# Enigmatisms/NeRF

Measured on AMD Instinct MI355X. Metric: rays/s (64+128 samples), 800x800, higher is better.
Workload: dtype bf16

## Files before the change

### nerf_amd/csrc/sample_kernels.hip

```cpp
#include "device_common.h"
#include "host_common.h"
#include "../../include/nerf_amd.h"

extern __shared__ __attribute__((aligned(16))) char smem[];

namespace {

constexpr int WAVES_PER_BLOCK = 4;

DEVINL int wave_in_block() { return (int)(threadIdx.x >> 6); }

constexpr int ENC_TILE = 64;
static inline size_t enc_lds_bytes(int L) { return (size_t)ENC_TILE * (6 * L + 6) * 4; }
template <bool IPE, class Moments>
DEVINL void encode_tile(float (*mom)[6], float* stage, int64_t base, int64_t total, int L, float* __restrict__ feat, Moments&& moments) {
    const int width = 6 * L, pairs_per = 3 * L;
    const int nsamp = (int)(total - base < ENC_TILE ? total - base : ENC_TILE);
    if ((int)threadIdx.x < nsamp) moments((int)threadIdx.x, base + threadIdx.x);
    __syncthreads();
    const int n_pairs = nsamp * pairs_per;
    for (int p = threadIdx.x; p < n_pairs; p += blockDim.x) {
        const int sl = p / pairs_per, rem = p - sl * pairs_per;
        const int l = rem / 3, c = rem - 3 * l;
        float sn, cs;
// ... 219 lines not shown
    for (int64_t n0 = blockIdx.x * (int64_t)4; n0 < N; n0 += (int64_t)gridDim.x * 4) {
        __syncthreads();
        if (threadIdx.x < 4 && n0 + threadIdx.x < N) {
            const int64_t n = n0 + threadIdx.x;
            const int64_t cell = (int64_t)__umul64hi(sampler_index_word(n, seed), P);
            const int64_t k = cell / wp, r = cell - k * wp;
            const int64_t wr = r / ww;
            const int64_t row = y0 + wr, col = x0 + (r - wr * ww);
            const int64_t v = view_ids != nullptr ? view_ids[k] : k;
            float* q = ray_s[threadIdx.x];
            if (v >= 0 && v < V) {
                sampler_ray(poses + v * 12, fx, fy, (float)(col - W / 2), (float)(H / 2 - row), q, rays + n * 6);
                const float* px = images + ((v * 3) * (int64_t)H + row) * W + col;
#pragma unroll
                for (int c = 0; c < 3; ++c) rgb[n * 3 + c] = px[(int64_t)c * H * W];
                if (index != nullptr) index[n] = (v * H + row) * W + col;
            } else {
                const float nan = __builtin_nanf("");
#pragma unroll
                for (int c = 0; c < 6; ++c) { q[c] = nan; rays[n * 6 + c] = nan; }
#pragma unroll
                for (int c = 0; c < 3; ++c) rgb[n * 3 + c] = nan;
                if (index != nullptr) index[n] = -1;
            }
        }
        __syncthreads();
        if (lengths == nullptr) continue;
        sampler_samples(n0, N, C, seed, near, res, ray_s, lengths, pts);
    }
}

__global__ void length2pts_kernel(const float* __restrict__ rays, const float* __restrict__ z, int64_t N, int S,
                                  float* __restrict__ out) {
    const int64_t total = N * S * 6;
    for (int64_t i = blockIdx.x * (int64_t)blockDim.x + threadIdx.x; i < total; i += (int64_t)gridDim.x * blockDim.x) {
        const int64_t ns = i / 6;
        const int k = (int)(i - ns * 6);
        const int64_t n = ns / S;
        const float* r = rays + n * 6;
        out[i] = (k < 3) ? (r[k] + r[3 + k] * z[ns]) : r[k];
    }
}

__global__ __launch_bounds__(256) void sigma_to_weights_kernel(const float* __restrict__ sigma, const float* __restrict__ z,
                                                              const float* __restrict__ dirs, int64_t N, int S, int act,
                                                              float* __restrict__ w) {
    for (int64_t n = blockIdx.x * (int64_t)WAVES_PER_BLOCK + wave_in_block(); n < N; n += (int64_t)gridDim.x * WAVES_PER_BLOCK) {
        float nrm = 1.0f;
        const bool scale = dirs != nullptr;
        if (scale) nrm = norm3(dirs[n * 3], dirs[n * 3 + 1], dirs[n * 3 + 2]);
        const float* sg = sigma + n * S;
        const float* zz = z + n * S;
        float* wo = w + n * S;
        wave_sigma_to_weights(S, act, [&](int s) { return sg[s]; },
                              [&](int s) { return scale ? zz[s] * nrm : zz[s]; },
                              [&](int s, float wv, float) { wo[s] = wv; });
    }
}

__global__ void max_blur_kernel(const float* __restrict__ w, int64_t N, int S, float alpha, float* __restrict__ out) {
    const int64_t total = N * S;
    for (int64_t i = blockIdx.x * (int64_t)blockDim.x + threadIdx.x; i < total; i += (int64_t)gridDim.x * blockDim.x) {
        const int s = (int)(i % S);
        const float c = w[i];
        const float front = (s == 0) ? c : fmaxf(w[i - 1], c);
        const float rear = (s == S - 1) ? c : fmaxf(c, w[i + 1]);
        out[i] = 0.5f * (front + rear) + alpha;
    }
}

DEVINL void lds_wave_sync() {
    __builtin_amdgcn_fence(__ATOMIC_RELEASE, "workgroup");
    __builtin_amdgcn_wave_barrier();
    __builtin_amdgcn_fence(__ATOMIC_ACQUIRE, "workgroup");
}

#ifndef SORT_NB_DEF
#define SORT_NB_DEF 256
#define SORT_CAP_DEF 6
#endif
constexpr int SORT_NB = SORT_NB_DEF, SORT_CAP = SORT_CAP_DEF, SORT_PER_LANE = SORT_NB / 64;
constexpr int SORT_LDS_FLOATS = 2 * SORT_NB + SORT_NB * SORT_CAP / 2;

template <class UF>
DEVINL void wave_inverse_sample(const float* pw, const float* bins, int nw, float* cdf, float* samp, int* bel, int* sortbuf,
                                UF&& uf, int K, int sort, float* __restrict__ z_out,
                                int64_t* __restrict__ below_out, int64_t* __restrict__ above_out) {
    const int lane = lane_id();
    const int nb = nw + 1;
    float* part8 = reinterpret_cast<float*>(sortbuf);
    const int nv = nw >> 3;
    if (lane < 8) {
        const int n4 = nv >> 2;
        float a0 = 0.0f, a1 = 0.0f, a2 = 0.0f, a3 = 0.0f;
        for (int i = 0; i < n4; ++i) {
            a0 += pw[32 * i + lane] + 1e-5f;
            a1 += pw[32 * i + 8 + lane] + 1e-5f;
            a2 += pw[32 * i + 16 + lane] + 1e-5f;
            a3 += pw[32 * i + 24 + lane] + 1e-5f;
        }
        for (int v = 4 * n4; v < nv; ++v) a0 += pw[8 * v + lane] + 1e-5f;
        a0 += a1; a0 += a2; a0 += a3;
        part8[lane] = a0;
    }
    lds_wave_sync();
    float total = 0.0f;
    if (nv > 0) {
        for (int j = 8 * nv; j < nw; ++j) total += pw[j] + 1e-5f;
#pragma unroll
        for (int c = 0; c < 8; ++c) total += part8[c];
    } else {
        float a1 = 0.0f, a2 = 0.0f, a3 = 0.0f;
        if (nw >= 4) { total += pw[0] + 1e-5f; a1 += pw[1] + 1e-5f; a2 += pw[2] + 1e-5f; a3 += pw[3] + 1e-5f; }
        for (int j = nw & ~3; j < nw; ++j) total += pw[j] + 1e-5f;
        total += a1; total += a2; total += a3;
    }
    double carry = 0.0;
    if (lane == 0) cdf[0] = 0.0f;
    for (int base = 0; base < nw; base += 64) {
        const int j = base + lane;
        double p = 0.0;
        if (j < nw) p = (double)((pw[j] + 1e-5f) / total);
        const double incl = wave_incl_scan_add(p);
        if (j < nw) cdf[1 + j] = (float)(carry + incl);
        carry += wave_last(incl);
    }
    lds_wave_sync();
    const int halvings = 32 - __builtin_clz((unsigned)nb);
    for (int k0 = 0, i0 = 0; k0 < K; k0 += 192, i0 += 3) {
        float uu[3]; int lo[3], hi[3];
#pragma unroll
        for (int q = 0; q < 3; ++q) {
            const int k = k0 + 64 * q + lane;
            uu[q] = (k < K) ? uf(i0 + q, k) : 0.0f;
            lo[q] = 0; hi[q] = (k < K) ? nb : 0;
        }
        for (int it = 0; it < halvings; ++it) {
#pragma unroll
            for (int q = 0; q < 3; ++q) {
                const int mid = (lo[q] + hi[q]) >> 1;
                const bool open_ = lo[q] < hi[q];
                const float c = cdf[open_ ? mid : 0];
                if (open_) { if (c <= uu[q]) lo[q] = mid + 1; else hi[q] = mid; }
            }
        }
#pragma unroll
        for (int q = 0; q < 3; ++q) {
            const int k = k0 + 64 * q + lane;
            if (k >= K) continue;
            const int below = lo[q] - 1 > 0 ? lo[q] - 1 : 0;
            const int above = lo[q] < nb - 1 ? lo[q] : nb - 1;
            const float c0 = cdf[below], c1 = cdf[above];
            float denom = c1 - c0;
            if (denom < 1e-5f) denom = 1.0f;
            const float t = (uu[q] - c0) / denom;
            const float b0 = bins[below], b1 = bins[above];
            const float v = b0 + t * (b1 - b0);
            if (sort) { samp[k] = v; bel[k] = below; }
            else {
                z_out[k] = v;
                if (below_out) below_out[k] = below;
                if (above_out) above_out[k] = above;
            }
        }
    }
    if (!sort) return;
    lds_wave_sync();
    int* cnt = sortbuf;
    int* pre = sortbuf + SORT_NB;
    unsigned short* mem = reinterpret_cast<unsigned short*>(sortbuf + 2 * SORT_NB);
    for (int b = lane; b < SORT_NB; b += 64) cnt[b] = 0;
    lds_wave_sync();
    int overflow = 0;
    for (int j = lane; j + 1 < nb; j += 64) overflow |= (bins[j + 1] < bins[j]) ? 1 : 0;
    for (int k = lane, i = 0; k < K; k += 64, ++i) {
        int b = (int)(uf(i, k) * (float)SORT_NB);
        b = b < 0 ? 0 : (b > SORT_NB - 1 ? SORT_NB - 1 : b);
        const int pos = atomicAdd(&cnt[b], 1);
        if (pos < SORT_CAP) mem[b * SORT_CAP + pos] = (unsigned short)k; else overflow = 1;
    }
    lds_wave_sync();
    if (__any(overflow)) {
        for (int k = lane; k < K; k += 64) {
            const float v = samp[k];
            int rank = 0;
            for (int j = 0; j < K; ++j) {
                const float o = samp[j];
                rank += (o < v || (o == v && j < k)) ? 1 : 0;
            }
            z_out[rank] = v;
            if (below_out) below_out[rank] = bel[k];
        }
        return;
    }
    {
        int c[SORT_PER_LANE], tot = 0;
#pragma unroll
        for (int i = 0; i < SORT_PER_LANE; ++i) { c[i] = cnt[lane * SORT_PER_LANE + i]; tot += c[i]; }
        int run = wave_incl_scan_add(tot) - tot;
#pragma unroll
        for (int i = 0; i < SORT_PER_LANE; ++i) { pre[lane * SORT_PER_LANE + i] = run; run += c[i]; }
    }
    lds_wave_sync();
    for (int k0 = 0, i0 = 0; k0 < K; k0 += 192, i0 += 3) {
        float v[3]; int rank[3], cntb[3], bb[3];
#pragma unroll
        for (int q = 0; q < 3; ++q) {
            const int k = k0 + 64 * q + lane;
            const bool ok = k < K;
            int b = ok ? (int)(uf(i0 + q, k) * (float)SORT_NB) : 0;
            b = b < 0 ? 0 : (b > SORT_NB - 1 ? SORT_NB - 1 : b);
            bb[q] = b;
            v[q] = samp[ok ? k : 0];
            rank[q] = pre[b];
            cntb[q] = ok ? cnt[b] : 0;
        }
        int most = cntb[0] > cntb[1] ? cntb[0] : cntb[1];
        most = most > cntb[2] ? most : cntb[2];
        const int trips = wave_max_i(most);
        for (int p = 0; p < trips; ++p) {
#pragma unroll
            for (int q = 0; q < 3; ++q) {
                const int k = k0 + 64 * q + lane;
                const bool live = p < cntb[q];
                const int jx = mem[bb[q] * SORT_CAP + p];
                const float o = samp[live ? jx : 0];
                rank[q] += (live && (o < v[q] || (o == v[q] && jx < k))) ? 1 : 0;
            }
        }
#pragma unroll
        for (int q = 0; q < 3; ++q) {
            const int k = k0 + 64 * q + lane;
            if (k >= K) continue;
            z_out[rank[q]] = v[q];
            if (below_out) below_out[rank[q]] = bel[k];
        }
    }
}

DEVINL size_t inv_lds_floats(int C, int K) { return (size_t)3 * C + 2 * K + SORT_LDS_FLOATS; }

__global__ __launch_bounds__(256) void inverse_sample_kernel(const float* __restrict__ w, const float* __restrict__ z,
                                                            const float* __restrict__ u, int64_t N, int C, int K, int sort,
                                                            int mode, float* __restrict__ z_out, int64_t* __restrict__ below,
                                                            int64_t* __restrict__ above) {
    float* base = reinterpret_cast<float*>(smem) + wave_in_block() * inv_lds_floats(C, K);
    float* pw = base; float* bins = pw + C; float* cdf = bins + C; float* samp = cdf + C;
    int* bel = reinterpret_cast<int*>(samp + K);
    int* sortbuf = bel + K;
    const int lane = lane_id();
    const int nw = mode == 0 ? C - 2 : C - 1;
    const int wstride = mode == 0 ? C : C - 1;
    for (int64_t n = blockIdx.x * (int64_t)WAVES_PER_BLOCK + wave_in_block(); n < N; n += (int64_t)gridDim.x * WAVES_PER_BLOCK) {
        lds_wave_sync();
        if (mode == 0) {
            for (int j = lane; j < nw; j += 64) pw[j] = w[n * wstride + 1 + j];
            for (int j = lane; j < nw + 1; j += 64) bins[j] = 0.5f * (z[n * C + j + 1] + z[n * C + j]);
        } else {
            for (int j = lane; j < nw; j += 64) pw[j] = w[n * wstride + j];
            for (int j = lane; j < nw + 1; j += 64) bins[j] = z[n * C + j];
        }
        lds_wave_sync();
        const float* un = u + n * K;
        wave_inverse_sample(pw, bins, nw, cdf, samp, bel, sortbuf, [&](int, int k) { return un[k]; }, K, sort, z_out + n * K,
                            below ? below + n * K : nullptr, above ? above + n * K : nullptr);
    }
}

struct ResampleArgs {
    const float* density; const float* z; const float* z_base; const float* u_strat; float z_jitter;
    const float* dirs; int dirs_stride; const float* u_inv; int64_t N; int C; int K; int softplus; float alpha;
    float* z_fine; int64_t* below; float* w_prop; float* z_coarse;
    uint64_t rng_seed; int64_t rng_ray_offset;
};

#ifndef RS_BLOCKS_PER_CU
#define RS_BLOCKS_PER_CU 5
#endif
__global__ __launch_bounds__(256) __attribute__((amdgpu_waves_per_eu(RS_BLOCKS_PER_CU, RS_BLOCKS_PER_CU))) void resample_kernel(ResampleArgs a) {
    const int C = a.C, K = a.K;
    float* base = reinterpret_cast<float*>(smem) + wave_in_block() * (inv_lds_floats(C, K) + 2 * C);
    float* pw = base; float* bins = pw + C; float* cdf = bins + C; float* samp = cdf + C;
    int* bel = reinterpret_cast<int*>(samp + K);
    int* sortbuf = bel + K;
    float* zl = reinterpret_cast<float*>(sortbuf + SORT_LDS_FLOATS);
    float* wraw = zl + C;
    const int lane = lane_id();
    struct RayIn { float dx, dy, dz, zv0, zv1, dens0, dens1, u0, u1, u2; };
    const bool fits = C <= 128 && K <= 192;
    auto load_in = [&](int64_t n) -> RayIn {
        RayIn r;
        const float* dd = a.dirs + n * a.dirs_stride;
        r.dx = dd[0]; r.dy = dd[1]; r.dz = dd[2];
        Philox4 blk = {{0u, 0u, 0u, 0u}};
        const bool draw = !a.u_inv || (!a.z && !a.u_strat);
        if (draw) blk = philox_ray_block(a.rng_seed, n + a.rng_ray_offset, lane);
        auto depth_of = [&](int j, bool first) {
            if (a.z) return a.z[n * C + j];
            const float uu = a.u_strat ? a.u_strat[n * C + j] : (first ? u01_from_bits(blk.w[0]) : philox_u_strat(a.rng_seed, n + a.rng_ray_offset, j));
            return a.z_base[j] + uu * a.z_jitter;
        };
        r.zv0 = r.zv1 = r.dens0 = r.dens1 = 0.0f;
        if (lane < C) { r.zv0 = depth_of(lane, true); r.dens0 = a.density[n * C + lane]; }
        if (lane + 64 < C) { r.zv1 = depth_of(lane + 64, false); r.dens1 = a.density[n * C + lane + 64]; }
        if (a.u_inv) {
            const float* un = a.u_inv + n * K;
            r.u0 = (lane < K) ? un[lane] : 0.0f;
            r.u1 = (lane + 64 < K) ? un[lane + 64] : 0.0f;
            r.u2 = (lane + 128 < K) ? un[lane + 128] : 0.0f;
        } else {
            r.u0 = u01_from_bits(blk.w[1]); r.u1 = u01_from_bits(blk.w[2]); r.u2 = u01_from_bits(blk.w[3]);
        }
        return r;
    };
    const int64_t stride = (int64_t)gridDim.x * WAVES_PER_BLOCK;
    int64_t n = blockIdx.x * (int64_t)WAVES_PER_BLOCK + wave_in_block();
    if (n >= a.N) return;
    RayIn cur = {};
    if (fits) cur = load_in(n);
    for (; n < a.N; n += stride) {
        RayIn nxt = cur;
        if (fits && n + stride < a.N) nxt = load_in(n + stride);
        lds_wave_sync();
        float nrm;
        if (fits) {
            nrm = norm3(cur.dx, cur.dy, cur.dz);
            if (lane < C) { zl[lane] = cur.zv0; if (a.z_coarse) a.z_coarse[n * C + lane] = cur.zv0; }
            if (lane + 64 < C) { zl[lane + 64] = cur.zv1; if (a.z_coarse) a.z_coarse[n * C + lane + 64] = cur.zv1; }
        } else {
            const float* dd = a.dirs + n * a.dirs_stride;
            nrm = norm3(dd[0], dd[1], dd[2]);
            for (int j = lane; j < C; j += 64) {
                const float zv = a.z ? a.z[n * C + j]
                                     : (a.z_base[j] + (a.u_strat ? a.u_strat[n * C + j] : philox_u_strat(a.rng_seed, n + a.rng_ray_offset, j)) * a.z_jitter);
                zl[j] = zv;
                if (a.z_coarse) a.z_coarse[n * C + j] = zv;
            }
        }
        lds_wave_sync();
        const float* sg = a.density + n * C;
        const int soft = a.softplus;
        const float dens0 = cur.dens0, dens1 = cur.dens1, cu0 = cur.u0, cu1 = cur.u1, cu2 = cur.u2;
        wave_sigma_to_weights(C, NERF_AMD_ACT_RELU,
                              [=](int s) { const float d = fits ? ((s >> 6) ? dens1 : dens0) : sg[s]; return soft ? softplus_f(d) : d; },
                              [=](int s) { return zl[s] * nrm; },
                              [=](int s, float wv, float) { wraw[s] = wv; });
        lds_wave_sync();
        for (int j = lane; j < C; j += 64) {
            const float c = wraw[j];
            const float front = (j == 0) ? c : fmaxf(wraw[j - 1], c);
            const float rear = (j == C - 1) ? c : fmaxf(c, wraw[j + 1]);
            const float wb = 0.5f * (front + rear) + a.alpha;
            if (j >= 1 && j <= C - 2) pw[j - 1] = wb;
            if (a.w_prop) a.w_prop[n * C + j] = wb;
        }
        for (int j = lane; j < C - 1; j += 64) bins[j] = 0.5f * (zl[j + 1] + zl[j]);
        lds_wave_sync();
        const float* un = a.u_inv ? a.u_inv + n * K : nullptr;
        const uint64_t seed = a.rng_seed; const int64_t nn = n + a.rng_ray_offset;
        wave_inverse_sample(pw, bins, C - 2, cdf, samp, bel, sortbuf,
                            [=](int i, int k) {
                                if (fits) return i == 0 ? cu0 : (i == 1 ? cu1 : cu2);
                                if (un) return un[k];
                                return philox_u_inv(seed, nn, k);
                            },
                            K, 1, a.z_fine + n * K, a.below ? a.below + n * K : nullptr, nullptr);
        cur = nxt;
    }
}

struct CompositeArgs {
    const float* rgbo; const float* z; int z_stride; const float* dirs; int dirs_stride; int64_t N; int S;
    int flags; int act; float sigma_shift; float near, far; const float* normal; const float* cam_dir;
    float* rgb; float* weights; float* depth; float* normal_img;
};

template <int NCH>
struct RayRecs { f32x4 c[NCH]; float z[NCH]; float dx, dy, dz; };
template <int NCH>
DEVINL RayRecs<NCH> load_ray(const CompositeArgs& a, int64_t n, int lane) {
    RayRecs<NCH> r;
    const f32x4 zero = {0.0f, 0.0f, 0.0f, 0.0f};
    const f32x4* px = reinterpret_cast<const f32x4*>(a.rgbo) + n * a.S;
    const float* zz = a.z + n * a.z_stride;
    const float* dd = a.dirs + n * a.dirs_stride;
#pragma unroll
    for (int k = 0; k < NCH; ++k) {
        const int s = 64 * k + lane;
        r.c[k] = (s < a.S) ? px[s] : zero;
        r.z[k] = (s < a.S) ? zz[s] : 0.0f;
    }
    r.dx = dd[0]; r.dy = dd[1]; r.dz = dd[2];
    return r;
}
template <int NCH>
DEVINL void composite_ray_fast(const CompositeArgs& a, int64_t n, const RayRecs<NCH>& r, int lane) {
    const int S = a.S;
    const bool mul = (a.flags & 1) != 0;
    const float nrm = mul ? norm3(r.dx, r.dy, r.dz) : 1.0f;
    float zn[NCH];
#pragma unroll
    for (int k = 0; k < NCH; ++k) zn[k] = mul ? r.z[k] * nrm : r.z[k];
    float accr = 0.0f, accg = 0.0f, accb = 0.0f, accw = 0.0f, accd = 0.0f;
    double carry = 1.0;
    float* wout = a.weights ? a.weights + n * S : nullptr;
#pragma unroll
    for (int k = 0; k < NCH; ++k) {
        if (k > 0 && 64 * k >= S) break;
        const int s = 64 * k + lane;
        float nx = __shfl_down(zn[k], 1, 64);
        if (k + 1 < NCH) { const float first = __shfl(zn[k + 1 < NCH ? k + 1 : k], 0, 64); if (lane == 63) nx = first; }
        float w = 0.0f;
        double p = 1.0;
        if (s < S) {
            const float delta = (s + 1 < S) ? (nx - zn[k]) : 1e10f;
            const float m = expf(-density_act(r.c[k][3] + a.sigma_shift, a.act) * delta);
            w = 1.0f - m; p = (double)(m + 1e-10f);
        }
        const double incl = wave_incl_scan_mul(p);
        const double excl = wave_shift_up1(incl, 1.0);
        w *= (float)(carry * excl);
        carry *= wave_last(incl);
        if (s < S) {
            accr += w * r.c[k][0]; accg += w * r.c[k][1]; accb += w * r.c[k][2]; accw += w; accd += w * zn[k];
            if (wout) wout[s] = w;
        }
    }
    accr = wave_sum(accr); accg = wave_sum(accg); accb = wave_sum(accb); accw = wave_sum(accw); accd = wave_sum(accd);
    if (lane == 0) {
        if (a.flags & 2) { const float bg = 1.0f - accw; accr += bg; accg += bg; accb += bg; }
        a.rgb[n * 3] = accr; a.rgb[n * 3 + 1] = accg; a.rgb[n * 3 + 2] = accb;
        if (a.depth) a.depth[n] = (accd - a.near) / (a.far - a.near);
    }
}
template <int NCH>
DEVINL void composite_rays_fast(const CompositeArgs& a, int lane) {
    const int64_t stride = (int64_t)gridDim.x * WAVES_PER_BLOCK;
    int64_t n = blockIdx.x * (int64_t)WAVES_PER_BLOCK + wave_in_block();
    if (n >= a.N) return;
    RayRecs<NCH> cur = load_ray<NCH>(a, n, lane);
    for (; n < a.N; n += stride) {
        RayRecs<NCH> nxt = cur;
        if (n + stride < a.N) nxt = load_ray<NCH>(a, n + stride, lane);
        composite_ray_fast<NCH>(a, n, cur, lane);
        cur = nxt;
    }
}

__global__ __launch_bounds__(256) void composite_kernel(CompositeArgs a) {
    const int S = a.S;
    const int lane = lane_id();
    if (S <= 256 && a.normal == nullptr && a.normal_img == nullptr) {
        if (S <= 128) composite_rays_fast<2>(a, lane);
        else composite_rays_fast<4>(a, lane);
        return;
    }
    for (int64_t n = blockIdx.x * (int64_t)WAVES_PER_BLOCK + wave_in_block(); n < a.N; n += (int64_t)gridDim.x * WAVES_PER_BLOCK) {
        const float* dd = a.dirs + n * a.dirs_stride;
        const bool mul = (a.flags & 1) != 0;
        const float nrm = mul ? norm3(dd[0], dd[1], dd[2]) : 1.0f;
        const float* zz = a.z + n * a.z_stride;
        const f32x4* px = reinterpret_cast<const f32x4*>(a.rgbo) + n * S;
        float accr = 0.0f, accg = 0.0f, accb = 0.0f, accw = 0.0f, accd = 0.0f, accn = 0.0f;
        float cx = 0.0f, cy = 0.0f, cz = 0.0f;
        if (a.normal_img) { cx = a.cam_dir[0]; cy = a.cam_dir[1]; cz = a.cam_dir[2]; }
        float* wout = a.weights ? a.weights + n * S : nullptr;
        const float* nm = a.normal ? a.normal + n * S * 3 : nullptr;
        const float shift = a.sigma_shift;
        wave_sigma_to_weights(S, a.act, [&](int s) { return px[s][3] + shift; },
                              [&](int s) { return mul ? zz[s] * nrm : zz[s]; },
                              [&](int s, float w, float zn) {
                                  const f32x4 c = px[s];
                                  accr += w * c[0]; accg += w * c[1]; accb += w * c[2];
                                  accw += w; accd += w * zn;
                                  if (nm) accn += w * ((nm[s * 3] * cx + nm[s * 3 + 1] * cy) + nm[s * 3 + 2] * cz);
                                  if (wout) wout[s] = w;
                              });
        accr = wave_sum(accr); accg = wave_sum(accg); accb = wave_sum(accb); accw = wave_sum(accw);
        accd = wave_sum(accd);
        if (a.normal_img) accn = wave_sum(accn);
        if (lane == 0) {
            if (a.flags & 2) { const float bg = 1.0f - accw; accr += bg; accg += bg; accb += bg; }
            a.rgb[n * 3] = accr; a.rgb[n * 3 + 1] = accg; a.rgb[n * 3 + 2] = accb;
            if (a.depth) a.depth[n] = (accd - a.near) / (a.far - a.near);
            if (a.normal_img) a.normal_img[n] = (accn + 1.0f) * 0.5f;
        }
    }
}

__global__ __launch_bounds__(256) void get_bounds_kernel(const float* __restrict__ w, const int64_t* __restrict__ below,
                                                        int64_t N, int C, int K, float* __restrict__ bounds) {
    float* sat = reinterpret_cast<float*>(smem) + wave_in_block() * (C + 1);
    const int lane = lane_id();
    for (int64_t n = blockIdx.x * (int64_t)WAVES_PER_BLOCK + wave_in_block(); n < N; n += (int64_t)gridDim.x * WAVES_PER_BLOCK) {
        lds_wave_sync();
        double carry = 0.0;
        if (lane == 0) sat[0] = 0.0f;
        for (int base = 0; base < C; base += 64) {
            const int j = base + lane;
            const double p = (j < C) ? (double)w[n * C + j] : 0.0;
            const double incl = wave_incl_scan_add(p);
            if (j < C) sat[1 + j] = (float)(carry + incl);
            carry += wave_last(incl);
        }
        lds_wave_sync();
        const int64_t* bl = below + n * K;
        for (int k = lane; k < K - 1; k += 64) {
            const int st = (int)bl[k], en = (int)bl[k + 1] + 1;
// ... 779 lines not shown
        const int64_t m = i >> 4;
        const int q = (int)(i & 15);
        float z[8];
        philox_normal8(seed, sample_offset + m, q, std, z);
        float* row = out + m * 128 + 16 * (q >> 1) + 4 * (q & 1);
        *reinterpret_cast<f32x4*>(row) = f32x4{z[0], z[1], z[2], z[3]};
        *reinterpret_cast<f32x4*>(row + 8) = f32x4{z[4], z[5], z[6], z[7]};
    }
}
int sk_philox_normal(float* out, int64_t M, uint64_t seed, const uint64_t* seed_dev, float std, int64_t sample_offset, hipStream_t st) {
    if (M == 0) return 0;
    hipLaunchKernelGGL(philox_normal_kernel, dim3(blocks_for(M * 16, 256)), dim3(256), 0, st, out, M, seed, seed_dev, std, sample_offset);
    return (int)hipGetLastError();
}
__global__ void advance_seed_kernel(uint64_t* __restrict__ seed_dev) {
    uint64_t x = seed_dev[0] + 0x9E3779B97F4A7C15ull;
    x = (x ^ (x >> 30)) * 0xBF58476D1CE4E5B9ull;
    x = (x ^ (x >> 27)) * 0x94D049BB133111EBull;
    seed_dev[0] = x ^ (x >> 31);
}
int sk_philox_uniforms(float* out, int64_t N, int K, uint64_t seed, const uint64_t* seed_dev, int64_t ray_offset, int strat, hipStream_t st) {
    if (N * K == 0) return 0;
    hipLaunchKernelGGL(philox_uniforms_kernel, dim3(blocks_for(N * K, 256)), dim3(256), 0, st, out, N, K, seed, seed_dev, ray_offset, strat);
    return (int)hipGetLastError();
}
int sk_advance_seed(uint64_t* seed_dev, hipStream_t st) {
    hipLaunchKernelGGL(advance_seed_kernel, dim3(1), dim3(1), 0, st, seed_dev);
    return (int)hipGetLastError();
}
int sk_generate_rays(const float* pose, int H, int W, float fx, float fy, int64_t first, int64_t count, float* rays,
                     hipStream_t st) {
    Cam c; c.H = H; c.W = W; c.fx = fx; c.fy = fy;
    for (int i = 0; i < 12; ++i) c.pose[i] = pose[i];
    if (count == 0) return 0;
    hipLaunchKernelGGL(raygen_kernel, dim3(blocks_for(count, 256)), dim3(256), 0, st, c, first, count, rays);
    return (int)hipGetLastError();
}
int sk_pixel_rays(const float* pose, float fx, float fy, const int64_t* coords, int64_t N, float* rays, hipStream_t st) {
    Cam c; c.H = 0; c.W = 0; c.fx = fx; c.fy = fy;
    for (int i = 0; i < 12; ++i) c.pose[i] = pose[i];
    if (N == 0) return 0;
    hipLaunchKernelGGL(pixel_rays_kernel, dim3(blocks_for(N, 256)), dim3(256), 0, st, c, coords, N, rays);
    return (int)hipGetLastError();
}
int sk_stratified_points(const float* rays, const float* z_base, const float* u, float jitter, int64_t N, int S, float* z_out,
                         float* pts, hipStream_t st) {
    if (N * S == 0) return 0;
    hipLaunchKernelGGL(stratified_points_kernel, dim3(blocks_for(N * S, 256)), dim3(256), 0, st, rays, z_base, u, jitter, N, S, z_out, pts);
    return (int)hipGetLastError();
}
int sk_length2pts(const float* rays, const float* z, int64_t N, int S, float* out, hipStream_t st) {
    if (N * S == 0) return 0;
    hipLaunchKernelGGL(length2pts_kernel, dim3(blocks_for(N * S * 6, 256)), dim3(256), 0, st, rays, z, N, S, out);
    return (int)hipGetLastError();
}
int sk_sigma_to_weights(const float* sigma, const float* z, const float* dirs, int64_t N, int S, int act, float* w, hipStream_t st) {
    if (N * S == 0) return 0;
    hipLaunchKernelGGL(sigma_to_weights_kernel, dim3(blocks_for(N, WAVES_PER_BLOCK)), dim3(256), 0, st, sigma, z, dirs, N, S, act, w);
    return (int)hipGetLastError();
}
int sk_max_blur(const float* w, int64_t N, int S, float alpha, float* out, hipStream_t st) {
    if (N * S == 0) return 0;
    hipLaunchKernelGGL(max_blur_kernel, dim3(blocks_for(N * S, 256)), dim3(256), 0, st, w, N, S, alpha, out);
    return (int)hipGetLastError();
}
int sk_inverse_sample(const float* w, const float* z, const float* u, int64_t N, int C, int K, int sort, int mode, float* z_out,
                      int64_t* below, int64_t* above, hipStream_t st) {
    if (N == 0) return 0;
    const size_t lds = WAVES_PER_BLOCK * ((size_t)3 * C + 2 * K + SORT_LDS_FLOATS) * 4;
    hipLaunchKernelGGL(inverse_sample_kernel, dim3(blocks_for(N, WAVES_PER_BLOCK)), dim3(256), lds, st, w, z, u, N, C, K, sort, mode,
                       z_out, below, above);
    return (int)hipGetLastError();
}
int sk_resample(const float* density, const float* z, const float* z_base, const float* u_strat, float z_jitter,
                const float* dirs, int dirs_stride, const float* u_inv, int64_t N, int C, int K, int softplus, float alpha,
                uint64_t rng_seed, int64_t rng_ray_offset, float* z_fine, int64_t* below, float* w_prop, float* z_coarse, hipStream_t st) {
    if (N == 0) return 0;
    ResampleArgs a{density, z, z_base, u_strat, z_jitter, dirs, dirs_stride, u_inv, N, C, K, softplus, alpha, z_fine, below, w_prop, z_coarse,
                   rng_seed, rng_ray_offset};
    const size_t lds = WAVES_PER_BLOCK * ((size_t)5 * C + 2 * K + SORT_LDS_FLOATS) * 4;
    int64_t blocks = (N + WAVES_PER_BLOCK - 1) / WAVES_PER_BLOCK;
    const int64_t resident = (int64_t)nerf_host::cu_count() * RS_BLOCKS_PER_CU;
    if (blocks > resident) blocks = resident;
    hipLaunchKernelGGL(resample_kernel, dim3((unsigned)blocks), dim3(256), lds, st, a);
    return (int)hipGetLastError();
}
int sk_composite(const float* rgbo, const float* z, int z_stride, const float* dirs, int dirs_stride, int64_t N, int S, int flags,
                 int act, float sigma_shift, float near, float far, const float* normal, const float* cam_dir, float* rgb, float* weights,
                 float* depth, float* normal_img, hipStream_t st) {
    if (N == 0) return 0;
    CompositeArgs a{rgbo, z, z_stride, dirs, dirs_stride, N, S, flags, act, sigma_shift, near, far, normal, cam_dir, rgb, weights, depth, normal_img};
    hipLaunchKernelGGL(composite_kernel, dim3(blocks_for(N, WAVES_PER_BLOCK)), dim3(256), 0, st, a);
    return (int)hipGetLastError();
}
int sk_get_bounds(const float* w, const int64_t* below, int64_t N, int C, int K, float* bounds, hipStream_t st) {
    if (N == 0 || K < 2) return 0;
    const size_t lds = WAVES_PER_BLOCK * ((size_t)C + 1) * 4;
    hipLaunchKernelGGL(get_bounds_kernel, dim3(blocks_for(N, WAVES_PER_BLOCK)), dim3(256), lds, st, w, below, N, C, K, bounds);
    return (int)hipGetLastError();
}

int sk_weights_backward(const float* sigma, int sigma_stride, int sigma_off, const float* z, int z_stride, const float* dirs, int dirs_stride,
                        int64_t N, int S, int mul_norm, int act, float sigma_shift, const float* rgbo, const float* d_rgb,
                        const float* d_weights, const float* d_depth, int white_bkg, float near, float far, float* d_sigma,
                        int d_sigma_stride, int d_sigma_off, float* d_rgbo, hipStream_t st) {
    if (N * S == 0) return 0;
    if (S > BWD_MAX_CHUNKS * 64) return (int)hipErrorInvalidValue;
    WeightsBwdArgs a{sigma, sigma_stride, sigma_off, z, z_stride, dirs, dirs_stride, N, S, mul_norm, act, sigma_shift, rgbo, d_rgb, d_weights,
                     d_depth, white_bkg, near, far, d_sigma, d_sigma_stride, d_sigma_off, d_rgbo};
    if (S <= 256) hipLaunchKernelGGL(weights_backward_kernel<4>, dim3(blocks_for(N, WAVES_PER_BLOCK)), dim3(256), 0, st, a);
    else if (S <= 512) hipLaunchKernelGGL(weights_backward_kernel<8>, dim3(blocks_for(N, WAVES_PER_BLOCK)), dim3(256), 0, st, a);
    else hipLaunchKernelGGL(weights_backward_kernel<16>, dim3(blocks_for(N, WAVES_PER_BLOCK)), dim3(256), 0, st, a);
    return (int)hipGetLastError();
}
int sk_max_blur_backward(const float* w, const float* g, int64_t N, int S, float* dw, hipStream_t st) {
    if (N * S == 0) return 0;
    hipLaunchKernelGGL(max_blur_backward_kernel, dim3(blocks_for(N * S, 256)), dim3(256), 0, st, w, g, N, S, dw);
    return (int)hipGetLastError();
}
int sk_get_bounds_backward(const int64_t* below, const float* g, int64_t N, int C, int K, float* dw, hipStream_t st) {
    if (N == 0) return 0;
    if (K < 2) { return (int)hipMemsetAsync(dw, 0, (size_t)N * C * 4, st); }
    const size_t lds = WAVES_PER_BLOCK * (size_t)(2 * K) * 4;
    hipLaunchKernelGGL(get_bounds_backward_kernel, dim3(blocks_for(N, WAVES_PER_BLOCK)), dim3(256), lds, st, below, g, N, C, K, dw);
    return (int)hipGetLastError();
}
int sk_frag_to_rows(const void* frag, int elem_bytes, int64_t n_sub, int n_kg, int64_t M, void* out, hipStream_t st) {
    if (n_sub == 0 || M == 0) return 0;
    const size_t lds = (size_t)WAVES_PER_BLOCK * 32 * ((size_t)n_kg * 16 * elem_bytes + 16);
    if (elem_bytes == 2) {
        hipLaunchKernelGGL(frag_to_rows_kernel<2>, dim3(blocks_for(n_sub, WAVES_PER_BLOCK)), dim3(256), lds, st, (const char*)frag, n_sub, n_kg, M, (char*)out, n_kg * 16);
    } else {
        if (int e = nerf_host::allow_dynamic_lds(reinterpret_cast<const void*>(frag_to_rows_kernel<4>), 140 * 1024)) return e;
        hipLaunchKernelGGL(frag_to_rows_kernel<4>, dim3(blocks_for(n_sub, WAVES_PER_BLOCK)), dim3(256), lds, st, (const char*)frag, n_sub, n_kg, M, (char*)out, n_kg * 16);
    }
    return (int)hipGetLastError();
}
int sk_relu_mask(void* delta, const void* act, int elem_bytes, int64_t n, hipStream_t st) {
    if (n == 0) return 0;
    const int64_t words = elem_bytes == 2 ? n / 2 : n;
    if (elem_bytes == 2) hipLaunchKernelGGL(relu_mask_kernel<2>, dim3(blocks_for(words, 256)), dim3(256), 0, st, (uint32_t*)delta, (const uint32_t*)act, words);
    else hipLaunchKernelGGL(relu_mask_kernel<4>, dim3(blocks_for(words, 256)), dim3(256), 0, st, (uint32_t*)delta, (const uint32_t*)act, words);
    return (int)hipGetLastError();
}
int sk_relu_mask_bias(void* delta, const void* act, int elem_bytes, int64_t rows, int cols, float* col_sum, hipStream_t st) {
    if (rows == 0) return 0;
    const int W = cols * elem_bytes / 4;
    if (W < 1 || W > 256 || (256 % W) != 0) return (int)hipErrorInvalidValue;
    const int rpb = 256 / W;
    int64_t blocks = (rows + rpb - 1) / rpb;
    if (blocks > 1024) blocks = 1024;
    if (elem_bytes == 2) hipLaunchKernelGGL(relu_mask_bias_kernel<2>, dim3((int)blocks), dim3(256), 0, st, (uint32_t*)delta, (const uint32_t*)act, rows, W, col_sum);
    else hipLaunchKernelGGL(relu_mask_bias_kernel<4>, dim3((int)blocks), dim3(256), 0, st, (uint32_t*)delta, (const uint32_t*)act, rows, W, col_sum);
    return (int)hipGetLastError();
}
int sk_merge_sorted(const float* a, const float* b, int64_t N, int K, int C, float* out, hipStream_t st) {
    if (N == 0) return 0;
    const size_t lds = WAVES_PER_BLOCK * (size_t)(K + C) * 2 * 4;
    hipLaunchKernelGGL(merge_sorted_kernel, dim3(blocks_for(N, WAVES_PER_BLOCK)), dim3(256), lds, st, a, b, N, K, C, out);
    return (int)hipGetLastError();
}
int sk_merge_sorted_order(const float* a, const float* b, const int64_t* f_inds, int64_t N, int K, int C, float* out, int64_t* order, int64_t* all_inds,
                          hipStream_t st) {
    if (N == 0) return 0;
    const size_t lds = WAVES_PER_BLOCK * (size_t)(K + C) * 4 * 4;
    hipLaunchKernelGGL(merge_sorted_order_kernel, dim3(blocks_for(N, WAVES_PER_BLOCK)), dim3(256), lds, st, a, b, f_inds, N, K, C, out, order, all_inds);
    return (int)hipGetLastError();
// ... 67 lines not shown
```

Baseline: 9.315 million.

## Specialize resample inverse sampling by slot count and add nontemporal composite loads

Splits the CDF construction into its own helper and adds a templated per-slot inverse sampler. The sampler is instantiated by the number of 64-wide sample slots, and it handles a small remainder of samples with ballot-based searches and wave-wide rank computation. The resample kernel becomes a template on slot count and fit, selected at launch, which removes runtime lambda branching and unused slot registers. The composite kernel also gets nontemporal loads and stores for streamed ray records and weights. The new path adds considerable complexity in the remainder ranking and overflow fallback.

```diff
diff --git a/nerf_amd/csrc/sample_kernels.hip b/nerf_amd/csrc/sample_kernels.hip
--- a/nerf_amd/csrc/sample_kernels.hip
+++ b/nerf_amd/csrc/sample_kernels.hip
@@ -325,13 +325,8 @@
 constexpr int SORT_NB = SORT_NB_DEF, SORT_CAP = SORT_CAP_DEF, SORT_PER_LANE = SORT_NB / 64;
 constexpr int SORT_LDS_FLOATS = 2 * SORT_NB + SORT_NB * SORT_CAP / 2;
 
-template <class UF>
-DEVINL void wave_inverse_sample(const float* pw, const float* bins, int nw, float* cdf, float* samp, int* bel, int* sortbuf,
-                                UF&& uf, int K, int sort, float* __restrict__ z_out,
-                                int64_t* __restrict__ below_out, int64_t* __restrict__ above_out) {
+DEVINL int wave_pdf_cdf(const float* pw, int nw, float* cdf, float* part8) {
     const int lane = lane_id();
-    const int nb = nw + 1;
-    float* part8 = reinterpret_cast<float*>(sortbuf);
     const int nv = nw >> 3;
     if (lane < 8) {
         const int n4 = nv >> 2;
@@ -359,16 +354,31 @@
         total += a1; total += a2; total += a3;
     }
     double carry = 0.0;
+    float prev_last = 0.0f;
+    int descends = 0;
     if (lane == 0) cdf[0] = 0.0f;
     for (int base = 0; base < nw; base += 64) {
         const int j = base + lane;
         double p = 0.0;
         if (j < nw) p = (double)((pw[j] + 1e-5f) / total);
         const double incl = wave_incl_scan_add(p);
-        if (j < nw) cdf[1 + j] = (float)(carry + incl);
+        const float c = (float)(carry + incl);
+        if (j < nw) cdf[1 + j] = c;
+        descends |= (j < nw && !(c >= dpp_move<DPP_WAVE_SHR1, 0xF>(prev_last, c))) ? 1 : 0;
+        prev_last = __builtin_bit_cast(float, __builtin_amdgcn_readlane(__builtin_bit_cast(int, c), 63));
         carry += wave_last(incl);
     }
     lds_wave_sync();
+    return descends;
+}
+
+template <class UF>
+DEVINL void wave_inverse_sample(const float* pw, const float* bins, int nw, float* cdf, float* samp, int* bel, int* sortbuf,
+                                UF&& uf, int K, int sort, float* __restrict__ z_out,
+                                int64_t* __restrict__ below_out, int64_t* __restrict__ above_out) {
+    const int lane = lane_id();
+    const int nb = nw + 1;
+    wave_pdf_cdf(pw, nw, cdf, reinterpret_cast<float*>(sortbuf));
     const int halvings = 32 - __builtin_clz((unsigned)nb);
     for (int k0 = 0, i0 = 0; k0 < K; k0 += 192, i0 += 3) {
         float uu[3]; int lo[3], hi[3];
@@ -481,6 +491,172 @@
     }
 }
 
+constexpr int SLOT_MAX_LEFT = 4;
+DEVINL int sort_bucket(float u) {
+    const int b = (int)(u * (float)SORT_NB);
+    return b < 0 ? 0 : (b > SORT_NB - 1 ? SORT_NB - 1 : b);
+}
+DEVINL float wave_bcast(float v, int src) { return __builtin_bit_cast(float, __builtin_amdgcn_readlane(__builtin_bit_cast(int, v), src)); }
+struct InvInterp { float v; int below; };
+DEVINL InvInterp inverse_interp(const float* cdf, const float* bins, int nb, int lo, float u) {
+    const int below = lo - 1 > 0 ? lo - 1 : 0;
+    const int above = lo < nb - 1 ? lo : nb - 1;
+    const float c0 = cdf[below], c1 = cdf[above];
+    float denom = c1 - c0;
+    if (denom < 1e-5f) denom = 1.0f;
+    const float t = (u - c0) / denom;
+    const float b0 = bins[below], b1 = bins[above];
+    return InvInterp{b0 + t * (b1 - b0), below};
+}
+template <int NS>
+DEVINL void wave_inverse_sample_slots(const float* pw, const float* bins, int nw, float* cdf, float* samp, int* bel, int* sortbuf,
+                                      float u0, float u1, float u2, int rem, int K, float* __restrict__ z_out,
+                                      int64_t* __restrict__ below_out) {
+    constexpr int NA = NS > 0 ? NS : 1;
+    const int lane = lane_id();
+    const int nb = nw + 1;
+    const bool ascending_cdf = !__any(wave_pdf_cdf(pw, nw, cdf, reinterpret_cast<float*>(sortbuf)));
+    const float us[3] = {u0, u1, u2};
+    const float ul = us[NS < 3 ? NS : 2];
+    float uu[NA], v[NA]; int lo[NA], hi[NA], bl[NA], bb[NA]; bool ok[NA];
+    const int halvings = 32 - __builtin_clz((unsigned)nb);
+#pragma unroll
+    for (int q = 0; q < NS; ++q) {
+        ok[q] = 64 * q + lane < K;
+        uu[q] = ok[q] ? us[q] : 0.0f;
+        lo[q] = 0; hi[q] = ok[q] ? nb : 0;
+    }
+    for (int it = 0; it < halvings; ++it) {
+#pragma unroll
+        for (int q = 0; q < NS; ++q) {
+            const int mid = (lo[q] + hi[q]) >> 1;
+            const bool open_ = lo[q] < hi[q];
+            const bool right = cdf[mid] <= uu[q];
+            lo[q] = (open_ & right) ? mid + 1 : lo[q];
+            hi[q] = (open_ & !right) ? mid : hi[q];
+        }
+    }
+#pragma unroll
+    for (int q = 0; q < NS; ++q) {
+        const InvInterp r = inverse_interp(cdf, bins, nb, lo[q], uu[q]);
+        v[q] = r.v; bl[q] = r.below;
+        bb[q] = sort_bucket(uu[q]);
+        if (ok[q]) samp[64 * q + lane] = v[q];
+    }
+    float lv[SLOT_MAX_LEFT] = {}; int lbl[SLOT_MAX_LEFT] = {}, lb[SLOT_MAX_LEFT] = {};
+    if (rem > 0) {
+        const float e0 = lane < nb ? cdf[lane] : 0.0f, e1 = lane + 64 < nb ? cdf[lane + 64] : 0.0f;
+#pragma unroll
+        for (int e = 0; e < SLOT_MAX_LEFT; ++e) {
+            if (e >= rem) continue;
+            const float u = wave_bcast(ul, e);
+            int l = 0;
+            if (ascending_cdf) {
+                l = __popcll(__ballot(lane < nb && e0 <= u)) + __popcll(__ballot(lane + 64 < nb && e1 <= u));
+            } else {
+                for (int h = nb; l < h;) {
+                    const int mid = (l + h) >> 1;
+                    if (cdf[mid] <= u) l = mid + 1; else h = mid;
+                }
+                l = __builtin_amdgcn_readfirstlane(l);
+            }
+            const InvInterp r = inverse_interp(cdf, bins, nb, l, u);
+            lv[e] = r.v; lbl[e] = r.below; lb[e] = sort_bucket(u);
+        }
+    }
+    lds_wave_sync();
+    int* cnt = sortbuf;
+    int* pre = sortbuf + SORT_NB;
+    unsigned short* mem = reinterpret_cast<unsigned short*>(sortbuf + 2 * SORT_NB);
+    for (int b = lane; b < SORT_NB; b += 64) cnt[b] = 0;
+    lds_wave_sync();
+    int overflow = 0;
+    for (int j = lane; j + 1 < nb; j += 64) overflow |= (bins[j + 1] < bins[j]) ? 1 : 0;
+#pragma unroll
+    for (int q = 0; q < NS; ++q) {
+        if (!ok[q]) continue;
+        const int pos = atomicAdd(&cnt[bb[q]], 1);
+        if (pos < SORT_CAP) mem[bb[q] * SORT_CAP + pos] = (unsigned short)(64 * q + lane); else overflow = 1;
+    }
+    lds_wave_sync();
+#pragma unroll
+    for (int e = 0; e < SLOT_MAX_LEFT; ++e) {
+        if (e >= rem) continue;
+        int members = cnt[lb[e]];
+#pragma unroll
+        for (int f = 0; f < SLOT_MAX_LEFT; ++f) members += (f < rem && lb[f] == lb[e]) ? 1 : 0;
+        overflow |= members > SORT_CAP ? 1 : 0;
+    }
+    if (__any(overflow)) {
+#pragma unroll
+        for (int q = 0; q < NS; ++q) if (ok[q]) bel[64 * q + lane] = bl[q];
+#pragma unroll
+        for (int e = 0; e < SLOT_MAX_LEFT; ++e)
+            if (e < rem && lane == 0) { samp[64 * NS + e] = lv[e]; bel[64 * NS + e] = lbl[e]; }
+        lds_wave_sync();
+        for (int k = lane; k < K; k += 64) {
+            const float val = samp[k];
+            int rank = 0;
+            for (int j = 0; j < K; ++j) {
+                const float o = samp[j];
+                rank += (o < val || (o == val && j < k)) ? 1 : 0;
+            }
+            z_out[rank] = val;
+            if (below_out) below_out[rank] = bel[k];
+        }
+        return;
+    }
+    {
+        int c[SORT_PER_LANE], tot = 0;
+#pragma unroll
+        for (int i = 0; i < SORT_PER_LANE; ++i) { c[i] = cnt[lane * SORT_PER_LANE + i]; tot += c[i]; }
+        int run = wave_incl_scan_add(tot) - tot;
+#pragma unroll
+        for (int i = 0; i < SORT_PER_LANE; ++i) { pre[lane * SORT_PER_LANE + i] = run; run += c[i]; }
+    }
+    lds_wave_sync();
+    int rank[NA], cntb[NA], most = 0;
+#pragma unroll
+    for (int q = 0; q < NS; ++q) {
+        rank[q] = pre[bb[q]];
+        cntb[q] = ok[q] ? cnt[bb[q]] : 0;
+        most = most > cntb[q] ? most : cntb[q];
+    }
+    const int trips = NS > 0 ? wave_max_i(most) : 0;
+    for (int p = 0; p < trips; ++p) {
+#pragma unroll
+        for (int q = 0; q < NS; ++q) {
+            const bool live = p < cntb[q];
+            const int jx = mem[bb[q] * SORT_CAP + p];
+            const float o = samp[live ? jx : 0];
+            rank[q] += (live & ((o < v[q]) | ((o == v[q]) & (jx < 64 * q + lane)))) ? 1 : 0;
+        }
+    }
+#pragma unroll
+    for (int e = 0; e < SLOT_MAX_LEFT; ++e) {
+        if (e >= rem) continue;
+        int ahead = 0;
+#pragma unroll
+        for (int q = 0; q < NS; ++q) {
+            ahead += __popcll(__ballot(ok[q] && (bb[q] < lb[e] || (bb[q] == lb[e] && v[q] <= lv[e]))));
+            rank[q] += (lb[e] < bb[q] || (lb[e] == bb[q] && lv[e] < v[q])) ? 1 : 0;
+        }
+#pragma unroll
+        for (int f = 0; f < SLOT_MAX_LEFT; ++f)
+            ahead += (f != e && f < rem && (lb[f] < lb[e] || (lb[f] == lb[e] && (lv[f] < lv[e] || (lv[f] == lv[e] && f < e))))) ? 1 : 0;
+        if (lane == 0) {
+            z_out[ahead] = lv[e];
+            if (below_out) below_out[ahead] = lbl[e];
+        }
+    }
+#pragma unroll
+    for (int q = 0; q < NS; ++q) {
+        if (!ok[q]) continue;
+        z_out[rank[q]] = v[q];
+        if (below_out) below_out[rank[q]] = bl[q];
+    }
+}
+
 DEVINL size_t inv_lds_floats(int C, int K) { return (size_t)3 * C + 2 * K + SORT_LDS_FLOATS; }
 
 __global__ __launch_bounds__(256) void inverse_sample_kernel(const float* __restrict__ w, const float* __restrict__ z,
@@ -520,8 +696,12 @@
 #ifndef RS_BLOCKS_PER_CU
 #define RS_BLOCKS_PER_CU 5
 #endif
+static inline int resample_left(int K) { return (K & 63) <= SLOT_MAX_LEFT ? (K & 63) : 0; }
+static inline int resample_slots(int K) { return (K - resample_left(K) + 63) / 64; }
+template <int NS, bool FITS>
 __global__ __launch_bounds__(256) __attribute__((amdgpu_waves_per_eu(RS_BLOCKS_PER_CU, RS_BLOCKS_PER_CU))) void resample_kernel(ResampleArgs a) {
     const int C = a.C, K = a.K;
+    const int rem = FITS && (K & 63) <= SLOT_MAX_LEFT ? (K & 63) : 0;
     float* base = reinterpret_cast<float*>(smem) + wave_in_block() * (inv_lds_floats(C, K) + 2 * C);
     float* pw = base; float* bins = pw + C; float* cdf = bins + C; float* samp = cdf + C;
     int* bel = reinterpret_cast<int*>(samp + K);
@@ -530,7 +710,7 @@
     float* wraw = zl + C;
     const int lane = lane_id();
     struct RayIn { float dx, dy, dz, zv0, zv1, dens0, dens1, u0, u1, u2; };
-    const bool fits = C <= 128 && K <= 192;
+    constexpr bool fits = FITS;
     auto load_in = [&](int64_t n) -> RayIn {
         RayIn r;
         const float* dd = a.dirs + n * a.dirs_stride;
@@ -599,15 +779,16 @@
         }
         for (int j = lane; j < C - 1; j += 64) bins[j] = 0.5f * (zl[j + 1] + zl[j]);
         lds_wave_sync();
-        const float* un = a.u_inv ? a.u_inv + n * K : nullptr;
-        const uint64_t seed = a.rng_seed; const int64_t nn = n + a.rng_ray_offset;
-        wave_inverse_sample(pw, bins, C - 2, cdf, samp, bel, sortbuf,
-                            [=](int i, int k) {
-                                if (fits) return i == 0 ? cu0 : (i == 1 ? cu1 : cu2);
-                                if (un) return un[k];
-                                return philox_u_inv(seed, nn, k);
-                            },
-                            K, 1, a.z_fine + n * K, a.below ? a.below + n * K : nullptr, nullptr);
+        if (fits) {
+            wave_inverse_sample_slots<NS>(pw, bins, C - 2, cdf, samp, bel, sortbuf, cu0, cu1, cu2, rem, K, a.z_fine + n * K,
+                                          a.below ? a.below + n * K : nullptr);
+        } else {
+            const float* un = a.u_inv ? a.u_inv + n * K : nullptr;
+            const uint64_t seed = a.rng_seed; const int64_t nn = n + a.rng_ray_offset;
+            wave_inverse_sample(pw, bins, C - 2, cdf, samp, bel, sortbuf,
+                                [=](int, int k) { return un ? un[k] : philox_u_inv(seed, nn, k); },
+                                K, 1, a.z_fine + n * K, a.below ? a.below + n * K : nullptr, nullptr);
+        }
         cur = nxt;
     }
 }
@@ -618,6 +799,11 @@
     float* rgb; float* weights; float* depth; float* normal_img;
 };
 
+#ifndef COMPOSITE_NT
+#define COMPOSITE_NT 1
+#endif
+DEVINL f32x4 stream_load(const f32x4* p) { return COMPOSITE_NT ? __builtin_nontemporal_load(p) : *p; }
+DEVINL void stream_store(float v, float* p) { if (COMPOSITE_NT) __builtin_nontemporal_store(v, p); else *p = v; }
 template <int NCH>
 struct RayRecs { f32x4 c[NCH]; float z[NCH]; float dx, dy, dz; };
 template <int NCH>
@@ -630,7 +816,7 @@
 #pragma unroll
     for (int k = 0; k < NCH; ++k) {
         const int s = 64 * k + lane;
-        r.c[k] = (s < a.S) ? px[s] : zero;
+        r.c[k] = (s < a.S) ? stream_load(px + s) : zero;
         r.z[k] = (s < a.S) ? zz[s] : 0.0f;
     }
     r.dx = dd[0]; r.dy = dd[1]; r.dz = dd[2];
@@ -666,7 +852,7 @@
         carry *= wave_last(incl);
         if (s < S) {
             accr += w * r.c[k][0]; accg += w * r.c[k][1]; accb += w * r.c[k][2]; accw += w; accd += w * zn[k];
-            if (wout) wout[s] = w;
+            if (wout) stream_store(w, wout + s);
         }
     }
     accr = wave_sum(accr); accg = wave_sum(accg); accb = wave_sum(accb); accw = wave_sum(accw); accd = wave_sum(accd);
@@ -1612,7 +1798,14 @@
     int64_t blocks = (N + WAVES_PER_BLOCK - 1) / WAVES_PER_BLOCK;
     const int64_t resident = (int64_t)nerf_host::cu_count() * RS_BLOCKS_PER_CU;
     if (blocks > resident) blocks = resident;
-    hipLaunchKernelGGL(resample_kernel, dim3((unsigned)blocks), dim3(256), lds, st, a);
+    const dim3 grid((unsigned)blocks), block(256);
+    if (C > 128 || K > 192) hipLaunchKernelGGL((resample_kernel<3, false>), grid, block, lds, st, a);
+    else switch (resample_slots(K)) {
+        case 0: hipLaunchKernelGGL((resample_kernel<0, true>), grid, block, lds, st, a); break;
+        case 1: hipLaunchKernelGGL((resample_kernel<1, true>), grid, block, lds, st, a); break;
+        case 2: hipLaunchKernelGGL((resample_kernel<2, true>), grid, block, lds, st, a); break;
+        default: hipLaunchKernelGGL((resample_kernel<3, true>), grid, block, lds, st, a); break;
+    }
     return (int)hipGetLastError();
 }
 int sk_composite(const float* rgbo, const float* z, int z_stride, const float* dirs, int dirs_stride, int64_t N, int S, int flags,
```

Result: no change. 9.340 million (median of 6 runs) (+0.3%).
